# rubengooj/stvo-pl

Measured on AMD Instinct MI355X. Metric: stereo frames/s (match+optimizePose), higher is better.
Workload: dtype u8/fp4+f64; 1 GPU; BASELINE configs[2]: KITTI-00-shaped stereo with points + lines (ORB + LBD rows), grid-windowed stereo match (points and lines) + f2f brute-force mutual-NNR match (points and lines) + full GN optimizePose (config_kitti.yaml), device-resident per-frame pipeline; the streams cycle through the 8 sequence ids / 3 KITTI calibrations of configs[4] (sequence s on rank s mod G); streams_per_gpu=3072, parallelism=seq-shard x1

## Files before the change

### stvo-pl_amd/csrc/match_kernels.hip

```cpp
#include "kernels.h"

#include <stdlib.h>

namespace stvo {

__device__ __forceinline__ uint32_t med3_u32(uint32_t a, uint32_t b, uint32_t c) {
    uint32_t r;
    asm("v_med3_u32 %0, %1, %2, %3" : "=v"(r) : "v"(a), "v"(b), "v"(c));
    return r;
}

__device__ __forceinline__ uint32_t bcnt_acc(uint32_t x, uint32_t acc) {
    uint32_t r;
    asm("v_bcnt_u32_b32 %0, %1, %2" : "=v"(r) : "v"(x), "v"(acc));
    return r;
}
__device__ __forceinline__ uint32_t pack_key(uint32_t d, uint32_t j_uniform) {
    uint32_t r;
    asm("v_lshl_or_b32 %0, %1, 16, %2" : "=v"(r) : "v"(d), "s"(j_uniform));
    return r;
}
__device__ __forceinline__ uint32_t bcnt0(uint32_t x) {
    uint32_t r;
    asm("v_bcnt_u32_b32 %0, %1, 0" : "=v"(r) : "v"(x));
// ... 174 lines not shown
    __shared__ int s_wave[4];
    const int b = blockIdx.x, tid = threadIdx.x, lane = tid & 63, wv = tid >> 6;
    const size_t off = (size_t)b * row_stride;
    const int nb = n2[b];
    const int per = (row_stride + 255) / 256;
    const int lo = tid * per, hi = min(lo + per, nb);
    int cnt = 0;
    for (int j = lo; j < hi; ++j) cnt += claim[off + j] != 0xFFFFFFFFu;
    int incl = cnt;
#pragma unroll
    for (int o = 1; o < 64; o <<= 1) {
        const int v = __shfl_up(incl, o, 64);
        if (lane >= o) incl += v;
    }
    if (lane == 63) s_wave[wv] = incl;
    __syncthreads();
    int base = 0, tot = 0;
#pragma unroll
    for (int w = 0; w < 4; ++w) {
        if (w < wv) base += s_wave[w];
        tot += s_wave[w];
    }
    int pos = base + incl - cnt;
    for (int j = lo; j < hi; ++j)
        if (claim[off + j] != 0xFFFFFFFFu) {
            qsel[off + pos++] = j;
            blocked[off + j] = 0;
        }
    if (tid == 0) nsel[b] = tot;
}

__device__ __forceinline__ uint32_t hamming128_lo(const uint4& q0, const uint32_t* __restrict__ t) {
    uint32_t d = bcnt0(q0.x ^ t[0]);
    d = bcnt_acc(q0.y ^ t[1], d);
    d = bcnt_acc(q0.z ^ t[2], d);
    d = bcnt_acc(q0.w ^ t[3], d);
    return d;
}
__device__ __forceinline__ uint32_t hamming128_hi(const uint4& q1, const uint32_t* __restrict__ t, uint32_t d) {
    d = bcnt_acc(q1.x ^ t[4], d);
    d = bcnt_acc(q1.y ^ t[5], d);
    d = bcnt_acc(q1.z ^ t[6], d);
    d = bcnt_acc(q1.w ^ t[7], d);
    return d;
}

__global__ __launch_bounds__(KNN_BLOCK) void hamming_verify_kernel(int B, int tiles, int nseg, int row_stride,
                                                                   const uint8_t* __restrict__ d1,
                                                                   const int32_t* __restrict__ n1,
                                                                   const uint8_t* __restrict__ d2,
                                                                   const uint32_t* __restrict__ claim,
                                                                   const int32_t* __restrict__ qsel,
                                                                   const int32_t* __restrict__ nsel, float nnr,
                                                                   int32_t* __restrict__ blocked) {
    const int per_frame = tiles * nseg;
    const int L = blockIdx.x;
    const int xcd = L & 7, k = L >> 3;
    const int b = (k / per_frame) * 8 + xcd;
    if (b >= B) return;
    const int local = k % per_frame;
    const int seg = local % nseg;
    const int tile = local / nseg;
    const int nq = nsel[b];
    const int nt_all = n1[b];
    const int seg_len = (((nt_all + nseg - 1) / nseg) + 3) & ~3;
    const int j0 = min(seg * seg_len, nt_all);
    const int nt = min(j0 + seg_len, nt_all);
    const int q_base = tile * KNN_BLOCK;
    if (q_base + (int)(threadIdx.x & ~63u) >= nq) return;
    const size_t frame_off = (size_t)b * row_stride;
    const uint32_t* __restrict__ T = reinterpret_cast<const uint32_t*>(d1 + frame_off * STVO_DESC_BYTES);

    const int q = q_base + threadIdx.x;
    const int qc = q < nq ? q : nq - 1;
    const int qi = qsel[frame_off + qc];
    const uint4 q0 = reinterpret_cast<const uint4*>(d2 + frame_off * STVO_DESC_BYTES)[2 * qi];
    const uint4 q1 = reinterpret_cast<const uint4*>(d2 + frame_off * STVO_DESC_BYTES)[2 * qi + 1];
    const uint32_t c = claim[frame_off + qi];
    const uint32_t istar = c & 0xFFFFu;
    uint32_t thr = c >> 16;
    {
        const float f0 = (float)thr;
        while (thr < 256u && !(f0 < (float)(thr + 1u) * nnr)) ++thr;
    }
    bool blk = false;
    auto step4 = [&](const uint32_t* __restrict__ t, int jb) {
        uint32_t p[4];
#pragma unroll
        for (int u = 0; u < 4; ++u) p[u] = hamming128_lo(q0, t + 8 * u);
        unsigned long long any = 0ull;
#pragma unroll
        for (int u = 0; u < 4; ++u) any |= __builtin_amdgcn_ballot_w64(p[u] <= thr);
        if (any != 0ull) {
            unsigned long long other = 0ull;
#pragma unroll
            for (int u = 0; u < 4; ++u) other |= __builtin_amdgcn_ballot_w64(p[u] <= thr && (uint32_t)(jb + u) != istar);
            if (other != 0ull) {
#pragma unroll
                for (int u = 0; u < 4; ++u) {
                    const uint32_t d = hamming128_hi(q1, t + 8 * u, p[u]);
                    blk = blk || (d <= thr && (uint32_t)(jb + u) != istar);
                }
            }
        }
    };
    int j = j0;
    if (j + 4 <= nt) {
        uint32_t ta[32], tb[32];
#pragma unroll
        for (int w = 0; w < 32; ++w) ta[w] = T[8 * j + w];
        for (; j + 8 <= nt; j += 8) {
#pragma unroll
            for (int w = 0; w < 32; ++w) tb[w] = T[8 * (j + 4) + w];
            step4(ta, j);
            const int jn = (j + 12 <= nt) ? j + 8 : j;
#pragma unroll
            for (int w = 0; w < 32; ++w) ta[w] = T[8 * jn + w];
            step4(tb, j + 4);
        }
        if (j + 4 <= nt) {
            step4(ta, j);
            j += 4;
        }
    }
    for (; j < nt; ++j) {
        const uint32_t d = hamming256(q0, q1, T + 8 * j);
        blk = blk || (d <= thr && (uint32_t)j != istar);
    }
    if (q < nq && blk) blocked[frame_off + qi] = 1;
}

__global__ __launch_bounds__(1024) void nnr_reverse_check_kernel(int row_stride, const uint32_t* __restrict__ claim,
                                                                 const int32_t* __restrict__ blocked, const int32_t* __restrict__ n1,
                                                                 int32_t* __restrict__ m12) {
    const int b = blockIdx.x;
    const size_t off = (size_t)b * row_stride;
    for (int i = threadIdx.x; i < row_stride; i += 1024) m12[off + i] = -1;
    __syncthreads();
    if (n1[b] < 2) return;
    for (int j = threadIdx.x; j < row_stride; j += 1024) {
        const uint32_t c = claim[off + j];
        if (c != 0xFFFFFFFFu && blocked[off + j] == 0) m12[off + (c & 0xFFFFu)] = j;
    }
}

__device__ __forceinline__ uint32_t block_threshold(uint32_t d0, float nnr) {
    const float f0 = (float)d0;
    uint32_t thr = d0;
    while (thr < 256u && !(f0 < (float)(thr + 1u) * nnr)) ++thr;
    return thr;
}

constexpr int PLAN_BLOCK = 512;
__global__ __launch_bounds__(PLAN_BLOCK) void forward_plan_kernel(int B, int nseg, int row_stride, uint2* __restrict__ knn12,
                                                                  const int32_t* __restrict__ n1,
                                                                  const int32_t* __restrict__ n2, float nnr,
                                                                  int32_t* __restrict__ m12, uint32_t* __restrict__ claim_g,
                                                                  int32_t* __restrict__ qsel, int32_t* __restrict__ tsel,
                                                                  int32_t* __restrict__ nsel) {
    extern __shared__ uint32_t plan_lds[];
    uint32_t* claim = plan_lds;
    uint16_t* Tc = reinterpret_cast<uint16_t*>(claim + row_stride);
    uint8_t* blk = reinterpret_cast<uint8_t*>(Tc + row_stride);
    __shared__ int hT[257], hS[257], s_cnt[3];
    __shared__ unsigned long long s_best;
    const int b = blockIdx.x, tid = threadIdx.x;
    const size_t off = (size_t)b * row_stride;
    const int na = n1[b], nb = n2[b];
    for (int j = tid; j < row_stride; j += PLAN_BLOCK) {
        claim[j] = 0xFFFFFFFFu;
        blk[j] = 0;
    }
    if (tid < 257) hT[tid] = hS[tid] = 0;
    if (tid < 3) s_cnt[tid] = 0;
    if (tid == 0) s_best = ~0ull;
    __syncthreads();
    const bool active = nb >= 2 && na >= 1;
    for (int i = tid; i < row_stride; i += PLAN_BLOCK) {
        if (active && i < na) {
            const uint2 k = merged_knn(knn12, (size_t)B * row_stride, off + i, nseg);
            if (nseg > 1) knn12[off + i] = k;
            const float f0 = (float)(k.x >> 16), f1 = (float)(k.y >> 16);
            if (f0 < f1 * nnr) atomicMin(&claim[k.x & 0xFFFFu], (k.x & 0xFFFF0000u) | (uint32_t)i);
        }
        m12[off + i] = -1;
    }
    __syncthreads();
    for (int j = tid; j < row_stride; j += PLAN_BLOCK) {
        const uint32_t c = claim[j];
        claim_g[off + j] = c;
        if (c != 0xFFFFFFFFu) {
            const uint32_t T = block_threshold(c >> 16, nnr);
            Tc[j] = (uint16_t)T;
            atomicAdd(&hT[T], 1);
        }
    }
    __syncthreads();
    if (active)
        for (int i = tid; i < na; i += PLAN_BLOCK) {
            const uint2 k = knn12[off + i];
            const uint32_t key[2] = {k.x, k.y};
#pragma unroll
            for (int e = 0; e < 2; ++e) {
                if (key[e] == 0xFFFFFFFFu) continue;
                const uint32_t j = key[e] & 0xFFFFu, c = claim[j];
                if (c != 0xFFFFFFFFu && (c & 0xFFFFu) != (uint32_t)i && (key[e] >> 16) <= (uint32_t)Tc[j]) blk[j] = 1;
            }
            if (k.y != 0xFFFFFFFFu) atomicAdd(&hS[min(k.y >> 16, 256u)], 1);
        }
    __syncthreads();
    if (tid < 64) {
        int vT[5], vS[5], sT = 0, sS = 0;
#pragma unroll
        for (int e = 0; e < 5; ++e) {
            const int t = tid * 5 + e;
            vT[e] = t < 257 ? hT[t] : 0;
            vS[e] = t < 257 ? hS[t] : 0;
            sT += vT[e];
            sS += vS[e];
        }
        int iT = sT, iS = sS;
#pragma unroll
        for (int o = 1; o < 64; o <<= 1) {
            const int a = __shfl_up(iT, o, 64), c = __shfl_up(iS, o, 64);
            if (tid >= o) {
                iT += a;
                iS += c;
            }
        }
        int eT = iT - sT, eS = iS - sS;
#pragma unroll
        for (int e = 0; e < 5; ++e) {
            const int t = tid * 5 + e;
            if (t < 257) {
                hT[t] = eT;
                hS[t] = eS;
            }
            eT += vT[e];
            eS += vS[e];
        }
        if (tid == 63) s_cnt[0] = iT;
    }
    __syncthreads();
    if (tid < 256) {
        const int C = s_cnt[0], cT = hT[tid], cS = hS[tid];
        const unsigned long long cost = (unsigned long long)(C - cT) * (unsigned)na + (unsigned long long)cT * (unsigned)cS;
        atomicMin(&s_best, (cost << 9) | (unsigned)tid);
    }
    __syncthreads();
    if (tid == 0) s_cnt[0] = 0;
    __syncthreads();
    const int tau = (int)(s_best & 511ull) - 1;
    for (int j = tid; j < row_stride; j += PLAN_BLOCK) {
        const uint32_t c = claim[j];
        if (c == 0xFFFFFFFFu) continue;
        if (!blk[j] && na >= 2) m12[off + (c & 0xFFFFu)] = j;
        if ((int)Tc[j] <= tau)
            qsel[off + atomicAdd(&s_cnt[0], 1)] = j;
        else
            qsel[off + row_stride - 1 - atomicAdd(&s_cnt[1], 1)] = j;
    }
    if (active)
        for (int i = tid; i < na; i += PLAN_BLOCK) {
            const uint2 k = knn12[off + i];
            if (k.y != 0xFFFFFFFFu && (int)(k.y >> 16) <= tau) tsel[off + atomicAdd(&s_cnt[2], 1)] = i;
        }
    __syncthreads();
    if (tid == 0) {
        nsel[b] = s_cnt[0] + s_cnt[1];
        nsel[(size_t)B + b] = s_cnt[0];
        nsel[2 * (size_t)B + b] = s_cnt[1];
        nsel[3 * (size_t)B + b] = s_cnt[2];
        nsel[4 * (size_t)B + b] = tau;
    }
}

struct ReversePlan {
    int32_t* tsel;
};
constexpr int KNN_REV_SLOTS = 4;
static ReversePlan reverse_plan(const LazyScratch& w, int B, int row_stride) {
    const size_t per = (size_t)B * row_stride;
    ReversePlan p;
    p.tsel = reinterpret_cast<int32_t*>(w.knn21 + (w.knn_capacity - per)) + per;
    return p;
}

static void launch_reverse_scans(hipStream_t s, int B, int row_stride, const uint8_t* d1, const int32_t* n1, const uint8_t* d2, float nnr,
                                 const LazyScratch& w, const ReversePlan& rp, int32_t* m12) {
    launch_hamming_knn2_mfma_reverse(s, B, row_stride, d1, n1, d2, w.qsel, w.nsel, rp.tsel, reinterpret_cast<const uint32_t*>(w.need), nnr, m12,
                                     KNN_REV_SLOTS);
}

void launch_hamming_verify(hipStream_t s, int B, int row_stride, const uint8_t* d1, const int32_t* n1, const uint8_t* d2,
                           float nnr, const LazyScratch& w, int lds_pad_bytes, int nseg, int32_t* m12) {
    if (B <= 0 || row_stride <= 0) return;
    const int mfma_qb = knn_mfma_qb(row_stride);
    if (mfma_qb > 0) {
        launch_reverse_scans(s, B, row_stride, d1, n1, d2, nnr, w, reverse_plan(w, B, row_stride), m12);
        return;
    }
    const int tiles = (row_stride + KNN_BLOCK - 1) / KNN_BLOCK, groups = (B + 7) / 8;
    hipLaunchKernelGGL(hamming_verify_kernel, dim3((unsigned)(groups * 8 * tiles * nseg)), dim3(KNN_BLOCK),
                       (size_t)lds_pad_bytes, s, B, tiles, nseg, row_stride, d1, n1, d2,
                       reinterpret_cast<const uint32_t*>(w.need), w.qsel, w.nsel, nnr, reinterpret_cast<int32_t*>(w.knn21));
}

void launch_match_mutual_lazy(hipStream_t s, int B, int row_stride, const uint8_t* d1, const int32_t* n1,
                              const uint8_t* d2, const int32_t* n2, float nnr, const LazyScratch& w, int32_t* m12,
                              int lds_pad_bytes, hipEvent_t wait_before_m12_write, hipEvent_t* tev) {
    if (B <= 0 || row_stride <= 0) return;
    const dim3 grid2((row_stride + 255) / 256, B);
    const int nseg = knn_pick_nseg(B, row_stride, w.knn_capacity);
    uint32_t* claim = reinterpret_cast<uint32_t*>(w.need);
    int32_t* blocked = reinterpret_cast<int32_t*>(w.knn21);
    if (tev) (void)hipEventRecord(tev[0], s);
    launch_hamming_knn2(s, B, row_stride, row_stride, d1, n1, d2, n2, w.knn12, w.knn21, 0, lds_pad_bytes, 0, nullptr,
                        nullptr, nseg, knn_mfma_qb(row_stride) > 0 ? nullptr : claim);
    if (tev) (void)hipEventRecord(tev[1], s);
    const int mfma_qb = knn_mfma_qb(row_stride);
    if (mfma_qb > 0) {
        const ReversePlan rp = reverse_plan(w, B, row_stride);
        if (wait_before_m12_write) (void)hipStreamWaitEvent(s, wait_before_m12_write, 0);
        if (tev && tev[2]) (void)hipEventRecord(tev[2], s);
        hipLaunchKernelGGL(forward_plan_kernel, dim3(B), dim3(PLAN_BLOCK), (size_t)row_stride * 7, s, B, nseg, row_stride, w.knn12,
                           n1, n2, nnr, m12, claim, w.qsel, rp.tsel, w.nsel);
        launch_reverse_scans(s, B, row_stride, d1, n1, d2, nnr, w, rp, m12);
        if (tev && tev[3]) (void)hipEventRecord(tev[3], s);
        return;
    }
    hipLaunchKernelGGL(nnr_forward_kernel, grid2, dim3(256), 0, s, nseg, row_stride, w.knn12, n1, n2, nnr, w.cand, claim);
    hipLaunchKernelGGL(compact_need_kernel, dim3(B), dim3(256), 0, s, row_stride, claim, n2, w.qsel, w.nsel, blocked);
    if (tev && tev[2]) (void)hipEventRecord(tev[2], s);
    launch_hamming_verify(s, B, row_stride, d1, n1, d2, nnr, w, lds_pad_bytes, nseg, m12);
    if (tev && tev[3]) (void)hipEventRecord(tev[3], s);
    if (wait_before_m12_write) (void)hipStreamWaitEvent(s, wait_before_m12_write, 0);
    hipLaunchKernelGGL(nnr_reverse_check_kernel, dim3(B), dim3(1024), 0, s, row_stride, claim, blocked, n1, m12);
}

const double kValuProbeOpsPerThreadIter = 19.0 * 8.0;

__global__ __launch_bounds__(256) void valu_probe_kernel(int iters, uint32_t* sink) {
    uint4 q0 = make_uint4(threadIdx.x * 2654435761u, blockIdx.x * 40503u + 1u, 0x9E3779B9u ^ threadIdx.x, 0x85EBCA6Bu);
    uint4 q1 = make_uint4(q0.y * 3u, q0.z * 5u, q0.w * 7u, q0.x * 11u);
    uint32_t best = 0xFFFFFFFFu, second = 0xFFFFFFFFu;
    uint32_t t[8];
    const uint32_t seed = __builtin_amdgcn_readfirstlane(blockIdx.x * 7919u + 13u);
#pragma unroll
    for (int k = 0; k < 8; ++k) t[k] = seed * (2 * k + 3);
    for (int it = 0; it < iters; ++it) {
#pragma unroll
        for (int u = 0; u < 8; ++u) {
#pragma unroll
            for (int k = 0; k < 8; ++k) t[k] = __builtin_amdgcn_readfirstlane(t[k] + 0x01010101u * (k + 1));
            const uint32_t d = hamming256(q0, q1, t);
            const uint32_t key = pack_key(d, (uint32_t)(it * 8 + u));
            second = med3_u32(best, second, key);
            best = best < key ? best : key;
        }
    }
    if ((best ^ second) == 0x12345u) sink[0] = best;
}

__global__ __launch_bounds__(256) void copy16_kernel(const uint4* __restrict__ src, uint4* __restrict__ dst, size_t n16) {
    for (size_t i = (size_t)blockIdx.x * 256 + threadIdx.x; i < n16; i += (size_t)gridDim.x * 256) dst[i] = src[i];
}

void launch_copy16(hipStream_t s, const void* src, void* dst, size_t bytes) {
    const size_t n16 = (bytes + 15) / 16;
    if (n16 == 0) return;
    const size_t blocks = (n16 + 255) / 256;
    hipLaunchKernelGGL(copy16_kernel, dim3((unsigned)(blocks < 256 ? blocks : 256)), dim3(256), 0, s,
                       reinterpret_cast<const uint4*>(src), reinterpret_cast<uint4*>(dst), n16);
}

void launch_valu_probe(hipStream_t s, int blocks, int iters, uint32_t* sink) {
    hipLaunchKernelGGL(valu_probe_kernel, dim3(blocks), dim3(256), 0, s, iters, sink);
}

__global__ __launch_bounds__(256) void match_small_kernel(int row_stride, int cap, const uint8_t* __restrict__ d1,
                                                          const int32_t* __restrict__ n1, const uint8_t* __restrict__ d2,
                                                          const int32_t* __restrict__ n2, float nnr, int mutual,
                                                          int32_t* __restrict__ m12) {
    extern __shared__ uint2 s_knn[];
    const int b = blockIdx.x, tid = threadIdx.x, lane = tid & 63;
    const int na = min(n1[b], cap), nb = min(n2[b], cap);
    const size_t off = (size_t)b * row_stride;
    uint2* k12 = s_knn;
    uint2* k21 = s_knn + cap;
    const int tiles_a = (na + 63) >> 6, tiles_b = mutual ? (nb + 63) >> 6 : 0;
    for (int item = tid >> 6; item < tiles_a + tiles_b; item += 4) {
        const int it = __builtin_amdgcn_readfirstlane(item);
        const bool fwd = it < tiles_a;
        const int q = (fwd ? it : it - tiles_a) * 64 + lane;
        const int nq = fwd ? na : nb, nt = fwd ? nb : na;
        const uint8_t* Q = (fwd ? d1 : d2) + off * STVO_DESC_BYTES;
        const uint32_t* __restrict__ T = reinterpret_cast<const uint32_t*>((fwd ? d2 : d1) + off * STVO_DESC_BYTES);
        const int qc = q < nq ? q : nq - 1;
        const uint4 q0 = reinterpret_cast<const uint4*>(Q)[2 * qc];
        const uint4 q1 = reinterpret_cast<const uint4*>(Q)[2 * qc + 1];
        uint32_t best = 0xFFFFFFFFu, second = 0xFFFFFFFFu;
        auto update = [&](uint32_t d, uint32_t jj) {
            const uint32_t key = pack_key(d, jj);
            second = med3_u32(best, second, key);
            best = best < key ? best : key;
        };
        int j = 0;
        for (; j + 4 <= nt; j += 4) {
            uint32_t t[32];
#pragma unroll
            for (int k = 0; k < 32; ++k) t[k] = T[8 * j + k];
            uint32_t d[4];
#pragma unroll
            for (int u = 0; u < 4; ++u) d[u] = hamming256(q0, q1, t + 8 * u);
#pragma unroll
            for (int u = 0; u < 4; ++u) update(d[u], (uint32_t)(j + u));
        }
        for (; j < nt; ++j) update(hamming256(q0, q1, T + 8 * j), (uint32_t)j);
        if (q < nq) (fwd ? k12 : k21)[q] = make_uint2(best, second);
    }
    __syncthreads();
    for (int i = tid; i < row_stride; i += 256) {
        int m = -1;
        if (i < na && nb >= 2) {
            const uint2 fk = k12[i];
            const float f0 = (float)(fk.x >> 16), f1 = (float)(fk.y >> 16);
            if (f0 < f1 * nnr) m = (int)(fk.x & 0xFFFFu);
            if (mutual && m >= 0) {
                bool keep = false;
                if (na >= 2) {
                    const uint2 rk = k21[m];
                    const float r0 = (float)(rk.x >> 16), r1 = (float)(rk.y >> 16);
                    keep = (r0 < r1 * nnr) && ((int)(rk.x & 0xFFFFu) == i);
                }
                if (!keep) m = -1;
            }
        }
        m12[off + i] = m;
    }
}

bool match_small_ok(int row_stride) { return row_stride > 0 && row_stride <= 512; }

void launch_match_small(hipStream_t s, int B, int row_stride, const uint8_t* d1, const int32_t* n1, const uint8_t* d2,
                        const int32_t* n2, float nnr, int mutual, int32_t* m12, int cap) {
    if (B <= 0 || !match_small_ok(row_stride)) return;
    if (cap <= 0 || cap > row_stride) cap = row_stride;
    const size_t lds = (size_t)cap * 2 * sizeof(uint2);
    hipLaunchKernelGGL(match_small_kernel, dim3(B), dim3(256), lds, s, row_stride, cap, d1, n1, d2, n2, nnr, mutual, m12);
}

}
```

### stvo-pl_amd/csrc/point_cells.h

```cpp
#pragma once

#include "kernels.h"

namespace stvo {

template <int T>
struct alignas(16) PointCellsLds {
    int lhist[GRID_LCELLS];
    int fill[STVO_GRID_CELLS];
    int hist[STVO_GRID_CELLS];
    int wave[T / 64];
    int extra;
};

template <int T, int N>
__device__ __forceinline__ int point_cells_scan(int* hist, int* s_wave, int32_t* start_out) {
    constexpr int PER = (N + T - 1) / T;
    constexpr bool FULL = N % T == 0;
    const int tid = threadIdx.x, lane = tid & 63, wv = tid >> 6;
    int local[PER];
    int sum = 0;
#pragma unroll
    for (int k = 0; k < PER; ++k) {
        const int c = tid * PER + k;
        local[k] = (FULL || c < N) ? hist[c] : 0;
        sum += local[k];
    }
    int incl = sum;
#pragma unroll
    for (int o = 1; o < 64; o <<= 1) {
        const int v = __shfl_up(incl, o, 64);
        if (lane >= o) incl += v;
    }
    if (lane == 63) s_wave[wv] = incl;
    __syncthreads();
    int base = 0, total = 0;
#pragma unroll
    for (int w = 0; w < T / 64; ++w) {
        const int c = s_wave[w];
        if (w < wv) base += c;
        total += c;
    }
    int run = base + incl - sum;
#pragma unroll
    for (int k = 0; k < PER; ++k) {
        const int c = tid * PER + k;
        if (FULL || c < N) {
            hist[c] = run;
            start_out[c] = run;
        }
        run += local[k];
    }
    if (tid == T - 1) start_out[N] = run;
    __syncthreads();
    return total;
}

__device__ __forceinline__ bool point_in_grid(int x, int y) {
    return x >= 0 && x < STVO_GRID_COLS && y >= 0 && y < STVO_GRID_ROWS;
}

template <int T, bool LEAN>
__device__ __forceinline__ void point_cells_frame(const PointCells& s, const int b, PointCellsLds<T>* lds) {
    constexpr int LPT = (2048 + T - 1) / T;
    int* hist = lds->hist;
    int* fill = lds->fill;
    int* lhist = lds->lhist;
    const int tid = threadIdx.x;
    const bool lsort = s.plperm != nullptr;
    const int nl = s.n_kp_l[b], nr = s.n_kp_r[b];
    const size_t off = (size_t)b * s.K;
    float2 rxy[LPT], lxy[LPT];
#pragma unroll
    for (int k = 0; k < LPT; ++k) rxy[k] = reinterpret_cast<const float2*>(s.kp_r)[off + min(tid + T * k, s.K - 1)];
#pragma unroll
    for (int k = 0; k < LPT; ++k) lxy[k] = reinterpret_cast<const float2*>(s.kp_l)[off + min(tid + T * k, s.K - 1)];
    __builtin_amdgcn_sched_barrier(0);
    const double inv_w = s.inv_wh[2 * b], inv_h = s.inv_wh[2 * b + 1];
    if (!LEAN)
        for (int i = tid; i < nl; i += T) {
            s.pxy_l[(off + i) * 2 + 0] = (int)((double)s.kp_l[(off + i) * 2 + 0] * inv_w);
            s.pxy_l[(off + i) * 2 + 1] = (int)((double)s.kp_l[(off + i) * 2 + 1] * inv_h);
        }
    for (int c = tid; c < STVO_GRID_CELLS; c += T) {
        hist[c] = 0;
        fill[c] = 0;
    }
    for (int c = tid; c < GRID_LCELLS; c += T) lhist[c] = 0;
    if (!LEAN)
        for (int i = tid; i < s.K; i += T) s.top2_p[off + i] = 0x00000000FFFFFFFFull;
    if (tid == 0) {
        if (!LEAN) s.govf_p[b] = 0;
        lds->extra = 0;
    }
    int rcel[LPT];
    {
#pragma unroll
        for (int k = 0; k < LPT; ++k) {
            const int x = (int)((double)rxy[k].x * inv_w);
            const int y = (int)((double)rxy[k].y * inv_h);
            rcel[k] = tid + T * k < nr ? (point_in_grid(x, y) ? y * STVO_GRID_COLS + x : -1) : -2;
        }
    }
    __syncthreads();
#pragma unroll
    for (int k = 0; k < LPT; ++k)
        if (rcel[k] >= 0) atomicAdd(&hist[rcel[k]], 1);
    for (int i = tid + T * LPT; i < nr; i += T) {
        const int x = (int)((double)s.kp_r[(off + i) * 2 + 0] * inv_w);
        const int y = (int)((double)s.kp_r[(off + i) * 2 + 1] * inv_h);
        if (point_in_grid(x, y)) atomicAdd(&hist[y * STVO_GRID_COLS + x], 1);
    }
    int lcel[LPT], lrnk[LPT];
    if (lsort) {
#pragma unroll
        for (int k = 0; k < LPT; ++k) {
            const int x = (int)((double)lxy[k].x * inv_w);
            const int y = (int)((double)lxy[k].y * inv_h);
            lcel[k] = (tid + T * k < nl && y >= 0 && y < STVO_GRID_ROWS && x >= 0 && x <= STVO_GRID_COLS - 1 + s.ws) ? y * GRID_LW + x : -1;
        }
#pragma unroll
        for (int k = 0; k < LPT; ++k) {
            lrnk[k] = 0;
            if (lcel[k] >= 0) lrnk[k] = atomicAdd(&lhist[lcel[k]], 1);
        }
    }
    __syncthreads();
    const int n_in = point_cells_scan<T, STVO_GRID_CELLS>(hist, lds->wave, s.pstart + (size_t)b * (STVO_GRID_CELLS + 1));
    if (lsort) {
        point_cells_scan<T, GRID_LCELLS>(lhist, lds->wave, reinterpret_cast<int32_t*>(s.plstart) + (size_t)b * GRID_LSTART_STRIDE);
#pragma unroll
        for (int k = 0; k < LPT; ++k)
            if (lcel[k] >= 0) s.plperm[off + lhist[lcel[k]] + lrnk[k]] = tid + T * k;
    }
    if (!LEAN)
        for (int i = tid; i < nl; i += T) {
            const int x = s.pxy_l[(off + i) * 2 + 0], y = s.pxy_l[(off + i) * 2 + 1];
            int lo = 0, hi = 0;
            if (y >= 0 && y < STVO_GRID_ROWS) {
                const int min_x = min(max(0, x - s.ws), STVO_GRID_COLS), max_x = max(min(STVO_GRID_COLS, x + 1), min_x);
                const int c0 = y * STVO_GRID_COLS + min_x, c1 = y * STVO_GRID_COLS + max_x;
                lo = c0 < STVO_GRID_CELLS ? hist[c0] : n_in;
                hi = c1 < STVO_GRID_CELLS ? hist[c1] : n_in;
            }
            s.prange[(off + i) * 2 + 0] = lo;
            s.prange[(off + i) * 2 + 1] = hi;
        }
    __syncthreads();
#pragma unroll
    for (int k = 0; k < LPT; ++k) {
        const int i = tid + T * k, c = rcel[k];
        if (c == -2) continue;
        int pos;
        if (c >= 0) {
            pos = hist[c] + atomicAdd(&fill[c], 1);
            if (!LEAN) s.pitems[off + pos] = i;
        } else {
            pos = n_in + atomicAdd(&lds->extra, 1);
        }
        s.pperm[off + pos] = i;
        s.pcell[off + pos] = c;
        if (!LEAN) s.prank[off + i] = pos;
    }
    for (int i = tid + T * LPT; i < nr; i += T) {
        const int x = (int)((double)s.kp_r[(off + i) * 2 + 0] * inv_w);
        const int y = (int)((double)s.kp_r[(off + i) * 2 + 1] * inv_h);
        const int c = point_in_grid(x, y) ? y * STVO_GRID_COLS + x : -1;
        int pos;
        if (c >= 0) {
            pos = hist[c] + atomicAdd(&fill[c], 1);
            if (!LEAN) s.pitems[off + pos] = i;
        } else {
            pos = n_in + atomicAdd(&lds->extra, 1);
        }
        s.pperm[off + pos] = i;
        s.pcell[off + pos] = c;
        if (!LEAN) s.prank[off + i] = pos;
    }
}

}
```

### stvo-pl_amd/csrc/seq_pipeline.hip

```cpp
#include <algorithm>
#include <atomic>
#include <chrono>
#include <cstdio>
#include <cstdlib>
#include <vector>

#include "ctx_internal.h"
#include "point_cells.h"
#include "pose_math.h"

#pragma clang fp contract(off)

namespace stvo {
namespace {

constexpr int LENT = STVO_GRID_COLS + STVO_GRID_ROWS + 4;

struct SeqDev {
    int B, K, M;
    const stvo_cam* cams;
    const double* inv_wh;
    stvo_match_params mp;
    const float* kp_l;
    const int32_t* oct_l;
// ... 83 lines not shown
}
template <typename T>
__device__ __forceinline__ void scan_cells(T* hist, int* s_wave, int32_t* start_out) {
    scan_cells_n<STVO_GRID_CELLS / 256>(hist, s_wave, start_out);
}

__host__ __device__ __forceinline__ PointCells point_cells_args(const SeqDev& s) {
    PointCells c;
    c.K = s.K; c.ws = s.mp.matching_s_ws;
    c.kp_l = s.kp_l; c.kp_r = s.kp_r; c.n_kp_l = s.n_kp_l; c.n_kp_r = s.n_kp_r; c.inv_wh = s.inv_wh;
    c.pstart = s.pstart; c.plstart = s.plstart; c.plperm = s.plperm; c.pperm = s.pperm; c.pcell = s.pcell;
    c.pxy_l = s.pxy_l; c.top2_p = s.top2_p; c.govf_p = s.govf_p; c.prange = s.prange; c.pitems = s.pitems; c.prank = s.prank;
    return c;
}
template <bool LEAN>
__global__ __launch_bounds__(256) void point_cells_kernel(SeqDev s) {
    __shared__ PointCellsLds<256> lds;
    point_cells_frame<256, LEAN>(point_cells_args(s), blockIdx.x, &lds);
}

constexpr int TAIL_BLOCK = 1024;
__host__ __device__ __forceinline__ PointTail point_tail_args(const SeqDev& s) {
    PointTail t;
    t.kp_l = s.kp_l; t.kp_r = s.kp_r; t.oct_l = s.oct_l; t.desc_l = s.desc_l; t.cams = s.cams;
    t.max_dist_epip = s.mp.max_dist_epip; t.min_disp = s.mp.min_disp;
    t.rc = s.rc; t.desc = s.desc; t.n = s.n; t.host_n = s.host_n; t.nl = s.nl; t.zero_nl = s.zero_nl;
    return t;
}
__global__ __launch_bounds__(TAIL_BLOCK) void point_tail_kernel(SeqDev s) {
    __shared__ int s_wave[TAIL_BLOCK / 64];
    __shared__ int s_run;
    const int b = blockIdx.x, tid = threadIdx.x, lane = tid & 63, wv = tid >> 6;
    const int nl = s.n_kp_l[b];
    const size_t off = (size_t)b * s.K;
    const PointTail t = point_tail_args(s);
    if (tid == 0) s_run = 0;
    __syncthreads();
    for (int base = 0; base < nl; base += TAIL_BLOCK) {
        const int i = base + tid;
        bool ok = false;
        double disp = 0.0;
        if (i < nl) {
            const int i2 = s.m12s_p[off + i];
            if (i2 >= 0) ok = point_tail_filter(t, off, i, i2, disp);
        }
        const unsigned long long bal = __ballot(ok);
        const int before = __popcll(bal & ((1ull << lane) - 1ull));
        if (lane == 0) s_wave[wv] = __popcll(bal);
        __syncthreads();
        int wbase = s_run;
        for (int w = 0; w < wv; ++w) wbase += s_wave[w];
        if (ok) point_tail_write(t, off, i, off + (size_t)(wbase + before), disp);
        __syncthreads();
        if (tid == 0) {
            int q = 0;
            for (int w = 0; w < TAIL_BLOCK / 64; ++w) q += s_wave[w];
            s_run += q;
        }
        __syncthreads();
    }
    if (tid == 0) {
        s.n[b] = s_run;
        if (s.host_n) s.host_n[b] = s_run;
        if (s.zero_nl) s.nl[b] = 0;
    }
}

template <typename F>
__device__ __forceinline__ void bresenham(double x1, double y1, double x2, double y2, F f) {
    const bool steep = fabs(y2 - y1) > fabs(x2 - x1);
    double t;
    if (steep) {
        t = x1; x1 = y1; y1 = t;
        t = x2; x2 = y2; y2 = t;
    }
    if (x1 > x2) {
        t = x1; x1 = x2; x2 = t;
        t = y1; y1 = y2; y2 = t;
    }
    const double dx = x2 - x1, dy = fabs(y2 - y1);
    double error = dx / 2.0;
    const int ystep = (y1 < y2) ? 1 : -1;
    int y = (int)y1;
    const int maxX = (int)x2;
    int guard = 0;
    for (int x = (int)x1; x <= maxX && guard < LENT; ++x, ++guard) {
        f(steep ? y : x, steep ? x : y);
        error -= dy;
        if (error < 0) {
            y += ystep;
            error += dx;
        }
    }
}

__global__ __launch_bounds__(256) void line_cells_kernel(SeqDev s) {
    __shared__ int hist[STVO_GRID_CELLS];
    __shared__ int fill[STVO_GRID_CELLS];
    __shared__ int s_wave[4];
    const int b = blockIdx.x, tid = threadIdx.x;
    const int nl = s.n_kl_l[b], nr = s.n_kl_r[b];
    const size_t off = (size_t)b * s.M;
    const double inv_w = s.inv_wh[2 * b], inv_h = s.inv_wh[2 * b + 1];
    for (int i = tid; i < nl; i += 256) {
        const float* kl = s.kl_l + (off + i) * 4;
        s.lxy_l[(off + i) * 4 + 0] = (int)((double)kl[0] * inv_w);
        s.lxy_l[(off + i) * 4 + 1] = (int)((double)kl[1] * inv_h);
        s.lxy_l[(off + i) * 4 + 2] = (int)((double)kl[2] * inv_w);
        s.lxy_l[(off + i) * 4 + 3] = (int)((double)kl[3] * inv_h);
    }
    for (int c = tid; c < STVO_GRID_CELLS; c += 256) {
        hist[c] = 0;
        fill[c] = 0;
    }
    __syncthreads();
    for (int j = tid; j < nr; j += 256) {
        const float* kl = s.kl_r + (off + j) * 4;
        const double vx = (double)(kl[2] - kl[0]) * inv_w;
        const double vy = (double)(kl[3] - kl[1]) * inv_h;
        const double mag = sqrt(vx * vx + vy * vy);
        s.ldir[(off + j) * 2 + 0] = vx / mag;
        s.ldir[(off + j) * 2 + 1] = vy / mag;
        s.lperm[off + j] = j;
        s.lrank[off + j] = j;
        bresenham((double)kl[0] * inv_w, (double)kl[1] * inv_h, (double)kl[2] * inv_w, (double)kl[3] * inv_h,
                  [&](int x, int y) {
                      if (in_grid(x, y)) atomicAdd(&hist[y * STVO_GRID_COLS + x], 1);
                  });
    }
    __syncthreads();
    scan_cells(hist, s_wave, s.lstart + (size_t)b * (STVO_GRID_CELLS + 1));
    int32_t* items = s.litems + (size_t)b * s.M * LENT;
    for (int j = tid; j < nr; j += 256) {
        const float* kl = s.kl_r + (off + j) * 4;
        bresenham((double)kl[0] * inv_w, (double)kl[1] * inv_h, (double)kl[2] * inv_w, (double)kl[3] * inv_h,
                  [&](int x, int y) {
                      if (in_grid(x, y)) {
                          const int c = y * STVO_GRID_COLS + x;
                          items[hist[c] + atomicAdd(&fill[c], 1)] = j;
                      }
                  });
    }
}

template <int T, typename MatchOf>
__device__ __forceinline__ void line_tail_frame(const SeqDev& s, const int b, MatchOf match_of, int* s_wave, int* s_run) {
    const int tid = threadIdx.x, lane = tid & 63, wv = tid >> 6;
    const int nl = s.n_kl_l[b];
    const size_t off = (size_t)b * s.M;
    const stvo_cam cam = s.cams[b];
    for (int base = 0; base < nl; base += T) {
        const int i = base + tid;
        bool ok = false;
        double sp_l[2] = {0, 0}, ep_l[2] = {0, 0}, le_l[3] = {0, 0, 0}, disp_s = 0.0, disp_e = 0.0;
        if (i < nl) {
            const int i2 = match_of(i);
            if (i2 >= 0) {
                const float* l = s.kl_l + (off + i) * 4;
                const float* r = s.kl_r + (off + i2) * 4;
                sp_l[0] = (double)l[0]; sp_l[1] = (double)l[1];
                ep_l[0] = (double)l[2]; ep_l[1] = (double)l[3];
                le_l[0] = sp_l[1] - ep_l[1];
                le_l[1] = ep_l[0] - sp_l[0];
                le_l[2] = sp_l[0] * ep_l[1] - sp_l[1] * ep_l[0];
                const double nrm = sqrt(le_l[0] * le_l[0] + le_l[1] * le_l[1]);
                le_l[0] /= nrm; le_l[1] /= nrm; le_l[2] /= nrm;
                double sp_r[2] = {(double)r[0], (double)r[1]}, ep_r[2] = {(double)r[2], (double)r[3]};
                const double overlap = pm::stereo_row_overlap(sp_l[1], ep_l[1], sp_r[1], ep_r[1], s.mp.line_horiz_th);
                sp_r[0] = (sp_r[0] * (sp_l[1] - ep_r[1]) + ep_r[0] * (sp_r[1] - sp_l[1])) / (sp_r[1] - ep_r[1]);
                sp_r[1] = sp_l[1];
                ep_r[0] = (sp_r[0] * (ep_l[1] - ep_r[1]) + ep_r[0] * (sp_r[1] - ep_l[1])) / (sp_r[1] - ep_r[1]);
                ep_r[1] = ep_l[1];
                pm::stereo_line_disparities(sp_l[0], ep_l[0], sp_r[0], ep_r[0], s.mp.ls_min_disp_ratio, &disp_s, &disp_e);
                ok = disp_s >= s.mp.min_disp && disp_e >= s.mp.min_disp && fabs(sp_l[1] - ep_l[1]) > s.mp.line_horiz_th &&
                     fabs(sp_r[1] - ep_r[1]) > s.mp.line_horiz_th && overlap > s.mp.stereo_overlap_th;
            }
        }
        const unsigned long long bal = __ballot(ok);
        const int before = __popcll(bal & ((1ull << lane) - 1ull));
        if (lane == 0) s_wave[wv] = __popcll(bal);
        __syncthreads();
        int wbase = (*s_run);
        for (int w = 0; w < wv; ++w) wbase += s_wave[w];
        if (ok) {
            const size_t k = off + (size_t)(wbase + before);
            const double bds = cam.b / disp_s, bde = cam.b / disp_e;
            s.spl[k * 2 + 0] = sp_l[0]; s.spl[k * 2 + 1] = sp_l[1];
            s.epl[k * 2 + 0] = ep_l[0]; s.epl[k * 2 + 1] = ep_l[1];
            s.sP[k * 3 + 0] = bds * (sp_l[0] - cam.cx);
            s.sP[k * 3 + 1] = bds * (sp_l[1] - cam.cy);
            s.sP[k * 3 + 2] = bds * cam.fx;
            s.eP[k * 3 + 0] = bde * (ep_l[0] - cam.cx);
            s.eP[k * 3 + 1] = bde * (ep_l[1] - cam.cy);
            s.eP[k * 3 + 2] = bde * cam.fx;
            s.le[k * 3 + 0] = le_l[0]; s.le[k * 3 + 1] = le_l[1]; s.le[k * 3 + 2] = le_l[2];
            const int level = s.oct_ll[off + i];
            double sg = 1.0;
            for (int t = 0; t < level; ++t) sg *= s.mp.lsd_scale;
            const double s2 = 1.0 / (sg * sg);
            s.s2l[k] = s2;
            double sm = s2;
            for (int t = 0; t < level; ++t) sm *= s.mp.lsd_scale;
            s.s2lm[k] = 1.0 / (sm * sm);
            const uint4* src = reinterpret_cast<const uint4*>(s.ldesc_l + (off + i) * STVO_DESC_BYTES);
            uint4* dst = reinterpret_cast<uint4*>(s.ldesc + k * STVO_DESC_BYTES);
            dst[0] = src[0];
            dst[1] = src[1];
        }
        __syncthreads();
        if (tid == 0)
            for (int w = 0; w < T / 64; ++w) (*s_run) += s_wave[w];
        __syncthreads();
    }
    if (tid == 0) {
        s.nl[b] = *s_run;
        if (s.host_nl) s.host_nl[b] = *s_run;
    }
}

__global__ __launch_bounds__(256) void line_tail_kernel(SeqDev s) {
    __shared__ int s_wave[4];
    __shared__ int s_run;
    const int b = blockIdx.x;
    const size_t off = (size_t)b * s.M;
    if (threadIdx.x == 0) s_run = 0;
    __syncthreads();
    line_tail_frame<256>(s, b, [&](int i) { return s.m12s_l[off + i]; }, s_wave, &s_run);
}

constexpr uint32_t LSF_ROW_EMPTY = 0xFFFFu;
constexpr uint32_t LSF_NO_WINDOW = 0x0000FFFFu;
constexpr int LSF_MAX_LINES = 512, LSF_BYTES_PER_LINE = 32 + 16 + 16 + 4 + 2 * STVO_GRID_ROWS + 2 + 2 + 1;
template <int T>
__global__ __launch_bounds__(T) void line_stereo_fused_kernel(SeqDev s, const int Mk, const int mutual, const double ratio) {
    extern __shared__ uint4 s_dyn[];
    __shared__ int s_wave[4];
    __shared__ int s_run;
    typedef uint32_t u32x4 __attribute__((ext_vector_type(4)));
    const int M = Mk, b = blockIdx.x, tid = threadIdx.x;
    u32x4* dl = reinterpret_cast<u32x4*>(s_dyn);
    int4* cxy = reinterpret_cast<int4*>(dl + 2 * M);
    double2* vdir = reinterpret_cast<double2*>(cxy + M);
    uint32_t* best = reinterpret_cast<uint32_t*>(vdir + M);
    unsigned short* rows = reinterpret_cast<unsigned short*>(best + M);
    unsigned short* owner = rows + (size_t)STVO_GRID_ROWS * M;
    short* mm = reinterpret_cast<short*>(owner + M);
    unsigned char* blocked = reinterpret_cast<unsigned char*>(mm + M);
    uint32_t* cand = reinterpret_cast<uint32_t*>(blocked + M + ((4 - (M & 3)) & 3));
    const int nl = min(s.n_kl_l[b], M), nr = min(s.n_kl_r[b], M);
    const size_t off = (size_t)b * s.M;
    const double inv_w = s.inv_wh[2 * b], inv_h = s.inv_wh[2 * b + 1];
    const int ws = s.mp.matching_s_ws;
    const double sim_th = s.mp.line_sim_th;
    if (tid == 0) s_run = 0;
    for (int i = tid; i < nl; i += T) {
        const float* kl = s.kl_l + (off + i) * 4;
        int4 c;
        c.x = (int)((double)kl[0] * inv_w);
        c.y = (int)((double)kl[1] * inv_h);
        c.z = (int)((double)kl[2] * inv_w);
        c.w = (int)((double)kl[3] * inv_h);
        auto window = [&](int x, int y, int& row_off, int& q) {
            const bool row_ok = y >= 0 && y < STVO_GRID_ROWS;
            const int lo = max(x - ws, 0), hi = min(x, STVO_GRID_COLS - 1);
            row_off = (row_ok ? y : 0) * M;
            q = (row_ok && lo <= hi) ? (int)((uint32_t)hi | ((uint32_t)(255 - lo) << 16)) : (int)LSF_NO_WINDOW;
        };
        int4 wq;
        window(c.x, c.y, wq.x, wq.y);
        window(c.z, c.w, wq.z, wq.w);
        cxy[i] = wq;
        const double vx = (double)(c.z - c.x), vy = (double)(c.w - c.y);
        const double mag = sqrt(vx * vx + vy * vy);
        vdir[i] = make_double2(vx / mag, vy / mag);
        const u32x4* g = reinterpret_cast<const u32x4*>(s.ldesc_l + (off + i) * STVO_DESC_BYTES);
        dl[2 * i] = g[0];
        dl[2 * i + 1] = g[1];
        best[i] = 0xFFFFFFFFu;
        blocked[i] = 0;
    }
    for (int j = tid; j < nr; j += T) {
        for (int y = 0; y < STVO_GRID_ROWS; ++y) rows[y * M + j] = (unsigned short)LSF_ROW_EMPTY;
        const float* kl = s.kl_r + (off + j) * 4;
        int cy = -1, cmn = 255, cmx = 0;
        auto flush = [&]() {
            if (cy >= 0 && cy < STVO_GRID_ROWS && cmn <= cmx) rows[cy * M + j] = (unsigned short)(cmn | ((255 - cmx) << 8));
        };
        bresenham((double)kl[0] * inv_w, (double)kl[1] * inv_h, (double)kl[2] * inv_w, (double)kl[3] * inv_h, [&](int x, int y) {
            if (y != cy) {
                flush();
                cy = y;
                cmn = 255;
                cmx = 0;
            }
            if (x >= 0 && x < STVO_GRID_COLS) {
                cmn = min(cmn, x);
                cmx = max(cmx, x);
            }
        });
        flush();
    }
    __syncthreads();
    typedef short i16x2 __attribute__((ext_vector_type(2)));
    auto in_window = [&](int j, int row_off, int q) -> bool {
        const uint32_t run = __builtin_amdgcn_perm(0u, (uint32_t)rows[row_off + j], 0x0c010c00u);
        const i16x2 d = __builtin_bit_cast(i16x2, q) - __builtin_bit_cast(i16x2, run);
        return (__builtin_bit_cast(uint32_t, d) & 0x80008000u) == 0u;
    };
    const int words = (nl + 31) >> 5;
    for (int e = tid; e < words * M; e += T) {
        const int w = e / M, j = e - w * M;
        uint32_t bits = 0u;
        if (j < nr) {
            const int i_end = min(32, nl - 32 * w);
#pragma unroll 4
            for (int k = 0; k < i_end; ++k) {
                const int4 c = cxy[32 * w + k];
                if (in_window(j, c.x, c.y) || in_window(j, c.z, c.w)) bits |= 1u << k;
            }
        }
        cand[e] = bits;
    }
    __syncthreads();
    auto walk = [&](int j, const u32x4 t0, const u32x4 t1, const double dirx, const double diry, auto f) {
        int run_min = 0x7FFFFFFF;
        for (int w = 0; w < words; ++w) {
            for (uint32_t bits = cand[w * M + j]; bits; bits &= bits - 1u) {
                const int i1 = 32 * w + __builtin_ctz(bits);
                const double2 v = vdir[i1];
                const double dot = v.x * dirx + v.y * diry;
                if (fabs(dot) < sim_th) continue;
                const u32x4 q0 = dl[2 * i1], q1 = dl[2 * i1 + 1];
                const int d = __builtin_popcount(q0.x ^ t0.x) + __builtin_popcount(q0.y ^ t0.y) + __builtin_popcount(q0.z ^ t0.z) +
                              __builtin_popcount(q0.w ^ t0.w) + __builtin_popcount(q1.x ^ t1.x) + __builtin_popcount(q1.y ^ t1.y) +
                              __builtin_popcount(q1.z ^ t1.z) + __builtin_popcount(q1.w ^ t1.w);
                if (mutual) {
                    if (d >= run_min) continue;
                    run_min = d;
                }
                f(i1, d);
            }
        }
    };
    auto right_line = [&](int j, u32x4& t0, u32x4& t1, double& dirx, double& diry) {
        const float* kl = s.kl_r + (off + j) * 4;
        const double vx = (double)(kl[2] - kl[0]) * inv_w;
        const double vy = (double)(kl[3] - kl[1]) * inv_h;
// ... 1107 lines not shown
```

Baseline: 1.389 million frame-pairs/s.

## Restructure forward match plan kernel with register keys and wave-aggregated slot allocation

Rewrites the forward plan kernel to keep merged knn keys in registers across phases when rows fit, replace the per-claim threshold array with a 257-entry LDS lookup table computed once via binary search, merge the histogram passes, and select tau with a wave shuffle reduction instead of LDS atomics plus extra barriers. qsel/tsel slot allocation now uses one atomic per wave with ballot/mbcnt, and m12 is written directly per row. Separately, line normal computation in the stereo line kernel is moved to only accepted lines, and the line cell sort packs cell and rank into one register. These aim to cut barriers, LDS atomics and register pressure, at the cost of a templated kernel and changed output ordering within qsel/tsel.

```diff
diff --git a/stvo-pl_amd/csrc/match_kernels.hip b/stvo-pl_amd/csrc/match_kernels.hip
--- a/stvo-pl_amd/csrc/match_kernels.hip
+++ b/stvo-pl_amd/csrc/match_kernels.hip
@@ -350,6 +350,41 @@
 }
 
 constexpr int PLAN_BLOCK = 512;
+constexpr int PLAN_ROWS = 4;
+
+__device__ __forceinline__ uint32_t plan_threshold(uint32_t d0, float nnr) {
+    const float f0 = (float)d0;
+    uint32_t lo = d0, hi = 256u;
+    while (lo < hi) {
+        const uint32_t mid = (lo + hi) >> 1;
+        if (f0 < (float)(mid + 1u) * nnr)
+            hi = mid;
+        else
+            lo = mid + 1u;
+    }
+    return lo;
+}
+
+__device__ __forceinline__ void plan_wave_slots(const bool (&take)[PLAN_ROWS], int* counter, int (&slot)[PLAN_ROWS]) {
+    unsigned long long m[PLAN_ROWS];
+    int total = 0;
+#pragma unroll
+    for (int r = 0; r < PLAN_ROWS; ++r) {
+        m[r] = __builtin_amdgcn_ballot_w64(take[r]);
+        total += __popcll(m[r]);
+    }
+    if (total == 0) return;
+    int base = 0;
+    if ((threadIdx.x & 63u) == 0u) base = atomicAdd(counter, total);
+    base = __builtin_amdgcn_readfirstlane(base);
+#pragma unroll
+    for (int r = 0; r < PLAN_ROWS; ++r) {
+        slot[r] = base + (int)__builtin_amdgcn_mbcnt_hi((uint32_t)(m[r] >> 32), __builtin_amdgcn_mbcnt_lo((uint32_t)m[r], 0u));
+        base += __popcll(m[r]);
+    }
+}
+
+template <bool REG>
 __global__ __launch_bounds__(PLAN_BLOCK) void forward_plan_kernel(int B, int nseg, int row_stride, uint2* __restrict__ knn12,
                                                                   const int32_t* __restrict__ n1,
                                                                   const int32_t* __restrict__ n2, float nnr,
@@ -358,53 +393,74 @@
                                                                   int32_t* __restrict__ nsel) {
     extern __shared__ uint32_t plan_lds[];
     uint32_t* claim = plan_lds;
-    uint16_t* Tc = reinterpret_cast<uint16_t*>(claim + row_stride);
-    uint8_t* blk = reinterpret_cast<uint8_t*>(Tc + row_stride);
-    __shared__ int hT[257], hS[257], s_cnt[3];
-    __shared__ unsigned long long s_best;
+    uint8_t* blk = reinterpret_cast<uint8_t*>(claim + row_stride);
+    __shared__ int hT[257], hS[257], s_cnt[3], s_tau;
+    __shared__ uint16_t s_thr[257];
+    constexpr int CHUNK = PLAN_ROWS * PLAN_BLOCK;
     const int b = blockIdx.x, tid = threadIdx.x;
     const size_t off = (size_t)b * row_stride;
     const int na = n1[b], nb = n2[b];
+    const bool active = nb >= 2 && na >= 1;
+    const uint2 no_key = make_uint2(0xFFFFFFFFu, 0xFFFFFFFFu);
+    uint2 kreg[PLAN_ROWS];
+#pragma unroll
+    for (int r = 0; r < PLAN_ROWS; ++r) kreg[r] = no_key;
+    if (REG && active) {
+#pragma unroll
+        for (int r = 0; r < PLAN_ROWS; ++r) {
+            const int i = tid + r * PLAN_BLOCK;
+            if (i < na) kreg[r] = merged_knn(knn12, (size_t)B * row_stride, off + i, nseg);
+        }
+    }
     for (int j = tid; j < row_stride; j += PLAN_BLOCK) {
         claim[j] = 0xFFFFFFFFu;
         blk[j] = 0;
     }
-    if (tid < 257) hT[tid] = hS[tid] = 0;
+    if (tid < 257) {
+        hT[tid] = hS[tid] = 0;
+        s_thr[tid] = (uint16_t)plan_threshold((uint32_t)tid, nnr);
+    }
     if (tid < 3) s_cnt[tid] = 0;
-    if (tid == 0) s_best = ~0ull;
     __syncthreads();
-    const bool active = nb >= 2 && na >= 1;
-    for (int i = tid; i < row_stride; i += PLAN_BLOCK) {
-        if (active && i < na) {
-            const uint2 k = merged_knn(knn12, (size_t)B * row_stride, off + i, nseg);
-            if (nseg > 1) knn12[off + i] = k;
-            const float f0 = (float)(k.x >> 16), f1 = (float)(k.y >> 16);
-            if (f0 < f1 * nnr) atomicMin(&claim[k.x & 0xFFFFu], (k.x & 0xFFFF0000u) | (uint32_t)i);
-        }
-        m12[off + i] = -1;
-    }
+    auto row_key = [&](int r, int i) -> uint2 {
+        if (REG) return kreg[r];
+        return (active && i < na) ? knn12[off + i] : no_key;
+    };
+    if (active)
+        for (int i0 = 0; i0 < (REG ? CHUNK : row_stride); i0 += CHUNK) {
+#pragma unroll
+            for (int r = 0; r < PLAN_ROWS; ++r) {
+                const int i = i0 + tid + r * PLAN_BLOCK;
+                if (i >= na) continue;
+                uint2 k = kreg[r];
+                if (!REG) k = merged_knn(knn12, (size_t)B * row_stride, off + i, nseg);
+                if (nseg > 1) knn12[off + i] = k;
+                const float f0 = (float)(k.x >> 16), f1 = (float)(k.y >> 16);
+                if (f0 < f1 * nnr) atomicMin(&claim[k.x & 0xFFFFu], (k.x & 0xFFFF0000u) | (uint32_t)i);
+                if (k.y != 0xFFFFFFFFu) atomicAdd(&hS[min(k.y >> 16, 256u)], 1);
+            }
+        }
     __syncthreads();
     for (int j = tid; j < row_stride; j += PLAN_BLOCK) {
         const uint32_t c = claim[j];
         claim_g[off + j] = c;
-        if (c != 0xFFFFFFFFu) {
-            const uint32_t T = block_threshold(c >> 16, nnr);
-            Tc[j] = (uint16_t)T;
-            atomicAdd(&hT[T], 1);
-        }
-    }
-    __syncthreads();
+        if (c != 0xFFFFFFFFu) atomicAdd(&hT[s_thr[c >> 16]], 1);
+    }
     if (active)
-        for (int i = tid; i < na; i += PLAN_BLOCK) {
-            const uint2 k = knn12[off + i];
-            const uint32_t key[2] = {k.x, k.y};
-#pragma unroll
-            for (int e = 0; e < 2; ++e) {
-                if (key[e] == 0xFFFFFFFFu) continue;
-                const uint32_t j = key[e] & 0xFFFFu, c = claim[j];
-                if (c != 0xFFFFFFFFu && (c & 0xFFFFu) != (uint32_t)i && (key[e] >> 16) <= (uint32_t)Tc[j]) blk[j] = 1;
+        for (int i0 = 0; i0 < (REG ? CHUNK : row_stride); i0 += CHUNK) {
+#pragma unroll
+            for (int r = 0; r < PLAN_ROWS; ++r) {
+                const int i = i0 + tid + r * PLAN_BLOCK;
+                if (i >= na) continue;
+                const uint2 k = row_key(r, i);
+                const uint32_t key[2] = {k.x, k.y};
+#pragma unroll
+                for (int e = 0; e < 2; ++e) {
+                    if (key[e] == 0xFFFFFFFFu) continue;
+                    const uint32_t j = key[e] & 0xFFFFu, c = claim[j];
+                    if (c != 0xFFFFFFFFu && (c & 0xFFFFu) != (uint32_t)i && (key[e] >> 16) <= (uint32_t)s_thr[c >> 16]) blk[j] = 1;
+                }
             }
-            if (k.y != 0xFFFFFFFFu) atomicAdd(&hS[min(k.y >> 16, 256u)], 1);
         }
     __syncthreads();
     if (tid < 64) {
@@ -426,50 +482,85 @@
                 iS += c;
             }
         }
+        const int C = __shfl(iT, 63, 64);
         int eT = iT - sT, eS = iS - sS;
+        unsigned long long best = ~0ull;
+        int bT = 0, bS = 0;
 #pragma unroll
         for (int e = 0; e < 5; ++e) {
             const int t = tid * 5 + e;
-            if (t < 257) {
-                hT[t] = eT;
-                hS[t] = eS;
+            if (t < 256) {
+                const unsigned long long cost = (unsigned long long)(C - eT) * (unsigned)na + (unsigned long long)eT * (unsigned)eS;
+                const unsigned long long cand = (cost << 9) | (unsigned)t;
+                if (cand < best) {
+                    best = cand;
+                    bT = eT;
+                    bS = eS;
+                }
             }
             eT += vT[e];
             eS += vS[e];
         }
-        if (tid == 63) s_cnt[0] = iT;
+        unsigned long long win = best;
+#pragma unroll
+        for (int o = 32; o > 0; o >>= 1) {
+            const unsigned long long other = __shfl_xor(win, o, 64);
+            win = other < win ? other : win;
+        }
+        if (win == best) {
+            const int tau = (int)(win & 511ull) - 1;
+            s_tau = tau;
+            nsel[b] = C;
+            nsel[(size_t)B + b] = bT;
+            nsel[2 * (size_t)B + b] = C - bT;
+            nsel[3 * (size_t)B + b] = bS;
+            nsel[4 * (size_t)B + b] = tau;
+        }
     }
     __syncthreads();
-    if (tid < 256) {
-        const int C = s_cnt[0], cT = hT[tid], cS = hS[tid];
-        const unsigned long long cost = (unsigned long long)(C - cT) * (unsigned)na + (unsigned long long)cT * (unsigned)cS;
-        atomicMin(&s_best, (cost << 9) | (unsigned)tid);
-    }
-    __syncthreads();
-    if (tid == 0) s_cnt[0] = 0;
-    __syncthreads();
-    const int tau = (int)(s_best & 511ull) - 1;
-    for (int j = tid; j < row_stride; j += PLAN_BLOCK) {
-        const uint32_t c = claim[j];
-        if (c == 0xFFFFFFFFu) continue;
-        if (!blk[j] && na >= 2) m12[off + (c & 0xFFFFu)] = j;
-        if ((int)Tc[j] <= tau)
-            qsel[off + atomicAdd(&s_cnt[0], 1)] = j;
-        else
-            qsel[off + row_stride - 1 - atomicAdd(&s_cnt[1], 1)] = j;
-    }
-    if (active)
-        for (int i = tid; i < na; i += PLAN_BLOCK) {
-            const uint2 k = knn12[off + i];
-            if (k.y != 0xFFFFFFFFu && (int)(k.y >> 16) <= tau) tsel[off + atomicAdd(&s_cnt[2], 1)] = i;
-        }
-    __syncthreads();
-    if (tid == 0) {
-        nsel[b] = s_cnt[0] + s_cnt[1];
-        nsel[(size_t)B + b] = s_cnt[0];
-        nsel[2 * (size_t)B + b] = s_cnt[1];
-        nsel[3 * (size_t)B + b] = s_cnt[2];
-        nsel[4 * (size_t)B + b] = tau;
+    const int tau = s_tau;
+    for (int j0 = 0; j0 < row_stride; j0 += CHUNK) {
+        bool lt[PLAN_ROWS], hv[PLAN_ROWS];
+        int sl[PLAN_ROWS], sh[PLAN_ROWS];
+#pragma unroll
+        for (int r = 0; r < PLAN_ROWS; ++r) {
+            const int j = j0 + tid + r * PLAN_BLOCK;
+            const uint32_t c = j < row_stride ? claim[j] : 0xFFFFFFFFu;
+            const bool claimed = c != 0xFFFFFFFFu;
+            const bool light = claimed && (int)s_thr[claimed ? c >> 16 : 0u] <= tau;
+            lt[r] = light;
+            hv[r] = claimed && !light;
+        }
+        plan_wave_slots(lt, &s_cnt[0], sl);
+        plan_wave_slots(hv, &s_cnt[1], sh);
+#pragma unroll
+        for (int r = 0; r < PLAN_ROWS; ++r) {
+            const int j = j0 + tid + r * PLAN_BLOCK;
+            if (lt[r]) qsel[off + sl[r]] = j;
+            if (hv[r]) qsel[off + row_stride - 1 - sh[r]] = j;
+        }
+    }
+    for (int i0 = 0; i0 < row_stride; i0 += CHUNK) {
+        bool in_s[PLAN_ROWS];
+        int ss[PLAN_ROWS];
+#pragma unroll
+        for (int r = 0; r < PLAN_ROWS; ++r) {
+            const int i = i0 + tid + r * PLAN_BLOCK;
+            const uint2 k = row_key(r, i);
+            in_s[r] = k.y != 0xFFFFFFFFu && (int)(k.y >> 16) <= tau;
+            if (i < row_stride) {
+                int m = -1;
+                if (k.x != 0xFFFFFFFFu && na >= 2) {
+                    const uint32_t j = k.x & 0xFFFFu;
+                    if (claim[j] == ((k.x & 0xFFFF0000u) | (uint32_t)i) && !blk[j]) m = (int)j;
+                }
+                m12[off + i] = m;
+            }
+        }
+        plan_wave_slots(in_s, &s_cnt[2], ss);
+#pragma unroll
+        for (int r = 0; r < PLAN_ROWS; ++r)
+            if (in_s[r]) tsel[off + ss[r]] = i0 + tid + r * PLAN_BLOCK;
     }
 }
 
@@ -521,8 +612,12 @@
         const ReversePlan rp = reverse_plan(w, B, row_stride);
         if (wait_before_m12_write) (void)hipStreamWaitEvent(s, wait_before_m12_write, 0);
         if (tev && tev[2]) (void)hipEventRecord(tev[2], s);
-        hipLaunchKernelGGL(forward_plan_kernel, dim3(B), dim3(PLAN_BLOCK), (size_t)row_stride * 7, s, B, nseg, row_stride, w.knn12,
-                           n1, n2, nnr, m12, claim, w.qsel, rp.tsel, w.nsel);
+        if (row_stride <= PLAN_ROWS * PLAN_BLOCK)
+            hipLaunchKernelGGL(forward_plan_kernel<true>, dim3(B), dim3(PLAN_BLOCK), (size_t)row_stride * 5, s, B, nseg, row_stride, w.knn12,
+                               n1, n2, nnr, m12, claim, w.qsel, rp.tsel, w.nsel);
+        else
+            hipLaunchKernelGGL(forward_plan_kernel<false>, dim3(B), dim3(PLAN_BLOCK), (size_t)row_stride * 5, s, B, nseg, row_stride, w.knn12,
+                               n1, n2, nnr, m12, claim, w.qsel, rp.tsel, w.nsel);
         launch_reverse_scans(s, B, row_stride, d1, n1, d2, nnr, w, rp, m12);
         if (tev && tev[3]) (void)hipEventRecord(tev[3], s);
         return;
diff --git a/stvo-pl_amd/csrc/point_cells.h b/stvo-pl_amd/csrc/point_cells.h
--- a/stvo-pl_amd/csrc/point_cells.h
+++ b/stvo-pl_amd/csrc/point_cells.h
@@ -111,19 +111,17 @@
         const int y = (int)((double)s.kp_r[(off + i) * 2 + 1] * inv_h);
         if (point_in_grid(x, y)) atomicAdd(&hist[y * STVO_GRID_COLS + x], 1);
     }
-    int lcel[LPT], lrnk[LPT];
+    int lpos[LPT];
     if (lsort) {
 #pragma unroll
         for (int k = 0; k < LPT; ++k) {
             const int x = (int)((double)lxy[k].x * inv_w);
             const int y = (int)((double)lxy[k].y * inv_h);
-            lcel[k] = (tid + T * k < nl && y >= 0 && y < STVO_GRID_ROWS && x >= 0 && x <= STVO_GRID_COLS - 1 + s.ws) ? y * GRID_LW + x : -1;
+            lpos[k] = (tid + T * k < nl && y >= 0 && y < STVO_GRID_ROWS && x >= 0 && x <= STVO_GRID_COLS - 1 + s.ws) ? y * GRID_LW + x : -1;
         }
 #pragma unroll
-        for (int k = 0; k < LPT; ++k) {
-            lrnk[k] = 0;
-            if (lcel[k] >= 0) lrnk[k] = atomicAdd(&lhist[lcel[k]], 1);
-        }
+        for (int k = 0; k < LPT; ++k)
+            if (lpos[k] >= 0) lpos[k] = (lpos[k] << 11) | atomicAdd(&lhist[lpos[k]], 1);
     }
     __syncthreads();
     const int n_in = point_cells_scan<T, STVO_GRID_CELLS>(hist, lds->wave, s.pstart + (size_t)b * (STVO_GRID_CELLS + 1));
@@ -131,7 +129,7 @@
         point_cells_scan<T, GRID_LCELLS>(lhist, lds->wave, reinterpret_cast<int32_t*>(s.plstart) + (size_t)b * GRID_LSTART_STRIDE);
 #pragma unroll
         for (int k = 0; k < LPT; ++k)
-            if (lcel[k] >= 0) s.plperm[off + lhist[lcel[k]] + lrnk[k]] = tid + T * k;
+            if (lpos[k] >= 0) s.plperm[off + lhist[lpos[k] >> 11] + (lpos[k] & 2047)] = tid + T * k;
     }
     if (!LEAN)
         for (int i = tid; i < nl; i += T) {
diff --git a/stvo-pl_amd/csrc/seq_pipeline.hip b/stvo-pl_amd/csrc/seq_pipeline.hip
--- a/stvo-pl_amd/csrc/seq_pipeline.hip
+++ b/stvo-pl_amd/csrc/seq_pipeline.hip
@@ -259,7 +259,7 @@
     for (int base = 0; base < nl; base += T) {
         const int i = base + tid;
         bool ok = false;
-        double sp_l[2] = {0, 0}, ep_l[2] = {0, 0}, le_l[3] = {0, 0, 0}, disp_s = 0.0, disp_e = 0.0;
+        double sp_l[2] = {0, 0}, ep_l[2] = {0, 0}, disp_s = 0.0, disp_e = 0.0;
         if (i < nl) {
             const int i2 = match_of(i);
             if (i2 >= 0) {
@@ -267,11 +267,6 @@
                 const float* r = s.kl_r + (off + i2) * 4;
                 sp_l[0] = (double)l[0]; sp_l[1] = (double)l[1];
                 ep_l[0] = (double)l[2]; ep_l[1] = (double)l[3];
-                le_l[0] = sp_l[1] - ep_l[1];
-                le_l[1] = ep_l[0] - sp_l[0];
-                le_l[2] = sp_l[0] * ep_l[1] - sp_l[1] * ep_l[0];
-                const double nrm = sqrt(le_l[0] * le_l[0] + le_l[1] * le_l[1]);
-                le_l[0] /= nrm; le_l[1] /= nrm; le_l[2] /= nrm;
                 double sp_r[2] = {(double)r[0], (double)r[1]}, ep_r[2] = {(double)r[2], (double)r[3]};
                 const double overlap = pm::stereo_row_overlap(sp_l[1], ep_l[1], sp_r[1], ep_r[1], s.mp.line_horiz_th);
                 sp_r[0] = (sp_r[0] * (sp_l[1] - ep_r[1]) + ep_r[0] * (sp_r[1] - sp_l[1])) / (sp_r[1] - ep_r[1]);
@@ -300,6 +295,12 @@
             s.eP[k * 3 + 0] = bde * (ep_l[0] - cam.cx);
             s.eP[k * 3 + 1] = bde * (ep_l[1] - cam.cy);
             s.eP[k * 3 + 2] = bde * cam.fx;
+            double le_l[3];
+            le_l[0] = sp_l[1] - ep_l[1];
+            le_l[1] = ep_l[0] - sp_l[0];
+            le_l[2] = sp_l[0] * ep_l[1] - sp_l[1] * ep_l[0];
+            const double nrm = sqrt(le_l[0] * le_l[0] + le_l[1] * le_l[1]);
+            le_l[0] /= nrm; le_l[1] /= nrm; le_l[2] /= nrm;
             s.le[k * 3 + 0] = le_l[0]; s.le[k * 3 + 1] = le_l[1]; s.le[k * 3 + 2] = le_l[2];
             const int level = s.oct_ll[off + i];
             double sg = 1.0;
```

Result: faster. 1.405 million frame-pairs/s (median of 6 runs) (+1.1%).
